# aras-p/UnityGaussianSplatting

Measured on AMD Instinct MI355X. Metric: Msplats/s rendered (sort+view+composite+resolve), bicycle-sized synthetic 6,131,954 splats, 1200x797, Medium; ms/frame in ms_per_step, higher is better.
Workload: dtype f32; 1 GPU; bicycle-sized synthetic 6,131,954 splats, 1200x797, Medium; sort_mode=visible_in_flight, frames_in_flight=2, frames_in_flight_impl=library, splats=6131954, views=1, views_per_rank=1, blend=exact, sort_nth_frame=1, tile_pairs_P=4376060, tile=32x16, visible_splats=1563698, parallelism=single GPU, rccl_ranks=0

## Files before the change

unitygaussiansplatting_amd/csrc/gs_common.h:

```cpp
#pragma once
#include <hip/hip_runtime.h>
#include <hip/hip_ext.h>
#include <stdint.h>
#include <stdio.h>
#include <string.h>
#include <utility>
#include <vector>

#include "../../include/gsplat_c.h"
#include "gs_device_math.h"
#include "gs_handles.h"
#include "gs_params.h"

#ifdef GS_CHAIN_PRIO
#define GS_CHAIN_PRIORITY() __builtin_amdgcn_s_setprio(GS_CHAIN_PRIO)
#else
#define GS_CHAIN_PRIORITY() do { } while (0)
#endif
#ifdef GS_VIEW_PRIO
#define GS_VIEW_PRIORITY() __builtin_amdgcn_s_setprio(GS_VIEW_PRIO)
#else
#define GS_VIEW_PRIORITY() do { } while (0)
#endif

namespace gs {

void set_error_detail(const char* fmt, ...);
int32_t fail(int32_t code, const char* what);
int32_t fail_hip(hipError_t e, const char* what, const char* file, int line);

#define GS_HIP(call)                                                        \
    do {                                                                    \
        hipError_t _e = (call);                                             \
        if (_e != hipSuccess) return gs::fail_hip(_e, #call, __FILE__, __LINE__); \
    } while (0)

#define GS_TRY(call)                    \
    do {                                \
        int32_t _r = (call);            \
        if (_r != GS_OK) return _r;     \
    } while (0)

constexpr int kBinThreads = 256;
constexpr int kBinItems = 8;
constexpr int kBinPart = kBinThreads * kBinItems;
constexpr uint32_t kBinTicketClasses = 16;
constexpr int kEvPerFrame = 28;

struct alignas(16) SplatRec {
    float cx, cy;
    float a1x, a1y;
    float a2x, a2y;
    uint32_t color0;
    uint32_t color1;
};
static_assert(sizeof(SplatRec) == 32, "SplatRec is 32 B");

struct ViewOutputs {
    gsm::ViewData* view;
    SplatRec* recs;
    uint2* rects;
    unsigned long long* visMask;
};
__host__ __device__ inline size_t vis_mask_words(uint32_t n) { return (((size_t)n + 63) / 64 + 7) & ~(size_t)7; }
__host__ __device__ inline uint8_t* wave_flags_of(unsigned long long* visMask, uint32_t n) { return (uint8_t*)(visMask + vis_mask_words(n)); }
__host__ __device__ inline size_t vis_alloc_bytes(uint32_t n) { return vis_mask_words(n) * 8 + ((size_t)n + 63) / 64 + 64; }

struct SortState {
    DevBuf<uint32_t> altKeys;
    DevBuf<uint32_t> altVals;
    DevBuf<uint32_t> status;
    DevBuf<unsigned long long> groupAgg;
    DevBuf<unsigned long long> groupIncl;
    uint32_t maxGroups = 0;
    uint32_t maxCount = 0;
    uint32_t maxParts = 0;
    uint32_t partMin = 8192;
    uint32_t histCopies = 1;
    uint32_t epoch = 0;
};

constexpr int kHistReplicas = 8;
constexpr int kHistStride = 4 * 256;
uint32_t hist_copies(int producerBlocks);
struct SortControl {
    uint32_t hist[kHistReplicas * kHistStride];
    uint32_t tickets[4][16 * 32];
    uint32_t error;
    uint32_t pad[3];
};

struct FrameReport {
    unsigned long long pairCount;
    uint32_t binError, pairSortError, visible, tileShape;
    uint32_t tieLongRuns, tieLongest;
};

constexpr int kVisHistory = 128;
constexpr uint32_t kVisMaxBlocks = 1024;
constexpr uint32_t kVisTieWaveMax = 64;
struct VisControl {
    uint32_t count;
    uint32_t tieLongRuns;
    uint32_t tieLongest;
    uint32_t error;
    uint32_t pad[28];
    uint32_t status[kVisMaxBlocks * 16];
};
constexpr uint32_t kVisStatusStride = 16;
struct TieHistory { float row[kVisHistory][4]; uint32_t depth; };
enum TieBase { TB_INDEX = 0,
               TB_RANK = 1,
               TB_POSITION = 2 };

struct alignas(16) PickRecord { float depth; uint32_t splat, tag, zero; };
static_assert(sizeof(PickRecord) == 16 && sizeof(PickRecord) == sizeof(gs_pick_record), "PickRecord is 16 B");
constexpr uint32_t kPickNoSplat = 0xFFFFFFFFu;
struct PickOut {
    PickRecord* rec;
    float tau;
    uint32_t tauHalfHi;
    uint32_t tag;
    uint32_t noDepth;
};

struct BinControl {
    unsigned long long pairCount;
    uint32_t pairCountClamped;
    uint32_t error;
    uint32_t tieLongRuns, tieLongest;
    uint32_t pad0[26];
    uint32_t visible;
    uint32_t pad1[31];
    uint32_t tickets[16 * 32];
};

}

struct gs_context {
    int device = 0;
    hipStream_t stream = nullptr;
    bool ownStream = false;
    hipStream_t aux = nullptr;
    bool overlap = false;
    gs::Event evOrder;
    bool viewGeneric = false;
    int sharedGpu = -1;
    bool counted = false;
    int cuCount = 0;
    hipDeviceProp_t props;
    std::vector<gs_context*> children;
    bool internalLane = false;
    bool sortBesideSiblings = false;
};
bool gs_shared_gpu(const gs_context* ctx);

struct gs_asset {
    gs_context* ctx = nullptr;
    gsm::AssetView view{};
    void* blobs[5] = {nullptr, nullptr, nullptr, nullptr, nullptr};
    gs::DevBuf<uint8_t> ownedBlobs[5];
    uint64_t sizes[5] = {0, 0, 0, 0, 0};
    bool owned = true;
};

struct gs_sorter {
    gs_context* ctx = nullptr;
    gs::SortState st;
    gs::DevBuf<gs::SortControl> control;
    gs::DevBuf<uint32_t> tmpKeys;
    gs::DevBuf<uint32_t> tmpVals;
};

struct gs_target {
    gs_context* ctx = nullptr;
    uint32_t width = 0, height = 0;
    gs::DevBuf<uint16_t> rgba16f;
    bool clearPending = false;
    const float* sceneDepth = nullptr;
    gs::DevBuf<float> sceneDepthOwned;
    gs::DevBuf<unsigned long long> zbuf;
    gs::DevBuf<float> resolved;
    gs::DevBuf<uint8_t> resolved8;
    static constexpr int kResolveRing = 64;
    std::vector<gs::Event> rev;
    bool profiling = false;
    int revCount = 0;
    gs::Event evLastUse;
    bool lastUseValid = false;
    gs::DevBuf<uint16_t> rgba16fAlt;
    gs::Event evLastUseAlt;
    bool lastUseValidAlt = false;
    bool exposed = false;
    gs::DevBuf<gs::PickRecord> pick;
    gs::DevBuf<gs::PickRecord> pickAlt;
    float pickTau = 0.5f;
};

struct gs_mask {
    gs_context* ctx = nullptr;
    uint32_t width = 0, height = 0, rowWords = 0;
    gs::DevBuf<uint32_t> words;
    gs::DevBuf<float> xy;
    gs::PinnedBuf<float> xyHost;
    gs::Event xyCopied;
    bool xyCopyPending = false;
    uint32_t xyCap = 0;
    gs::PinnedBuf<uint32_t> wordsHost;
    gs::Event wordsCopied;
    bool wordsCopyPending = false;
};

namespace gs {
struct RendererSettings {
    int blendMode = 0;
    int renderMode = 0;
    float pointDisplaySize = 3.0f;
    bool alwaysWriteView = false;
    bool kernelTiming = false;
// ... 243 lines not shown
```

unitygaussiansplatting_amd/csrc/gs_device_math.h:

```cpp
#pragma once
#include <stdint.h>

#if defined(__HIPCC__)
#include <hip/hip_runtime.h>
#include <hip/hip_fp16.h>
#define GS_HD __host__ __device__ __forceinline__
#else
#include <cmath>
#include <cstring>
#define GS_HD inline
#endif

#ifndef GS_CULL_EXTENT
#define GS_CULL_EXTENT 2.8285f
#endif

namespace gsm {

struct AssetView {
    const uint8_t* pos;
    const uint8_t* other;
    const uint8_t* color;
    const uint8_t* sh;
    const uint8_t* chunk;
// ... 874 lines not shown
            return s;
        };
        auto MUL = [](float w, const RGB& s) -> RGB { return { F2{ w, w } * s.rg, w * s.b }; };
        auto FMA = [](float w, const RGB& s, const RGB& acc) -> RGB { return { fma2(F2{ w, w }, s.rg, acc.rg), fmaf(w, s.b, acc.b) }; };
        {
            const RGB s1v = SHK(1), s2v = SHK(2), s3v = SHK(3);
            RGB t = MUL(dy, RGB{ -s1v.rg, -s1v.b });
            t = FMA(dz, s2v, t);
            t = FMA(dx, RGB{ -s3v.rg, -s3v.b }, t);
            rg = fma2(F2{ GS_SH_C1, GS_SH_C1 }, t.rg, rg); b = fmaf(GS_SH_C1, t.b, b);
        }
        if (P.shOrder >= 2) {
            const float xx = dx * dx, yy = dy * dy, zz = dz * dz;
            const float xy = dx * dy, yz = dy * dz, xz = dx * dz;
            {
                const float b4 = 1.0925484f * xy, b5 = -1.0925484f * yz, b6 = 0.3153916f * (fmaf(2.0f, zz, -xx) - yy),
                            b7 = -1.0925484f * xz, b8 = 0.5462742f * (xx - yy);
                RGB acc = MUL(b4, SHK(4));
                acc = FMA(b5, SHK(5), acc);
                acc = FMA(b6, SHK(6), acc);
                acc = FMA(b7, SHK(7), acc);
                acc = FMA(b8, SHK(8), acc);
                rg += acc.rg; b += acc.b;
            }
            if (P.shOrder >= 3) {
                const float b9 = (-0.5900436f * dy) * fmaf(3.0f, xx, -yy);
                const float b10 = (2.8906114f * xy) * dz;
                const float b11 = (-0.4570458f * dy) * (fmaf(4.0f, zz, -xx) - yy);
                const float b12 = (0.3731763f * dz) * (fmaf(2.0f, zz, -3.0f * xx) - 3.0f * yy);
                const float b13 = (-0.4570458f * dx) * (fmaf(4.0f, zz, -xx) - yy);
                const float b14 = (1.4453057f * dz) * (xx - yy);
                const float b15 = (-0.5900436f * dx) * fmaf(-3.0f, yy, xx);
                RGB acc = MUL(b9, SHK(9));
                acc = FMA(b10, SHK(10), acc);
                acc = FMA(b11, SHK(11), acc);
                acc = FMA(b12, SHK(12), acc);
                acc = FMA(b13, SHK(13), acc);
                acc = FMA(b14, SHK(14), acc);
                acc = FMA(b15, SHK(15), acc);
                rg += acc.rg; b += acc.b;
            }
        }
    }
    float r = rg.x, g = rg.y;
    r = fmaxf(r, 0.0f); g = fmaxf(g, 0.0f); b = fmaxf(b, 0.0f);
    view.color[0] = (f32tof16(r) << 16) | f32tof16(g);
    view.color[1] = (f32tof16(b) << 16) | (view.color[1] & 0xffffu);
}

template <class SHSource>
GS_HD ViewData CalcViewDataT(const AssetView& a, const FrameConsts& P, const EditView& E, uint32_t idx, SHSource& shsrc) {
    ViewPartial vp;
    CalcViewGeom(a, P, E, idx, vp);
    if (vp.front) CalcViewColor(a, P, idx, vp, shsrc);
    return vp.view;
}

GS_HD ViewData CalcViewData(const AssetView& a, const FrameConsts& P, const EditView& E, uint32_t idx) {
    SHFromBlob src;
    return CalcViewDataT(a, P, E, idx, src);
}

GS_HD void PixRange(float c, float e, float size, int& lo, int& hi) {
    float flo = ceilf((c - e) - 0.5f), fhi = floorf((c + e) - 0.5f);
    flo = fmaxf(flo, 0.0f); fhi = fminf(fhi, size - 1.0f);
    if (!(flo <= fhi)) { lo = 1; hi = 0; return; }
    lo = (int)flo; hi = (int)fhi;
}

constexpr uint32_t kAlphaThresholdBits = 0x3B808081u;
constexpr uint32_t kAlphaWindow = 16u;
constexpr uint32_t kAlphaWindowLo = kAlphaThresholdBits - kAlphaWindow / 2u;
GS_HD float Exp2Det(float y) {
    const float n = rintf(y);
    const float f = y - n;
    float p = 1.525273380405984e-05f;
    p = fmaf(p, f, 1.5403530393381608e-04f);
    p = fmaf(p, f, 1.3333558146428443e-03f);
    p = fmaf(p, f, 9.618129107628477e-03f);
    p = fmaf(p, f, 5.550410866482158e-02f);
    p = fmaf(p, f, 2.402265069591007e-01f);
    p = fmaf(p, f, 6.931471805599453e-01f);
    p = fmaf(p, f, 1.0f);
    return ldexpf(p, (int)n);
}
GS_HD float DecideAlpha(float alphaNative, float y, float a, bool& live) {
    const uint32_t u = f2u(alphaNative) - kAlphaWindowLo;
    if (u < kAlphaWindow) {
        const float ad = fminf(fmaxf(Exp2Det(y) * a, 0.0f), 1.0f);
        live = ad >= u2f(kAlphaThresholdBits);
        return ad;
    }
    live = (int32_t)u >= (int32_t)kAlphaWindow;
    return alphaNative;
}

constexpr uint32_t kSelRingLoBits = 0x3CE0E0E1u;
constexpr uint32_t kSelRingHiBits = 0x3D20A0A1u;
GS_HD bool SplatSelected(const EditView& E, uint32_t idx) { return E.selectedBits && ((E.selectedBits[idx >> 5] >> (idx & 31u)) & 1u); }
constexpr uint32_t kSelectedAlphaHalf = 0xBC00u;
GS_HD bool SelectedNearThreshold(float eNative) {
    const uint32_t b = f2u(eNative), h = kAlphaWindow / 2u;
    return (b - (kAlphaThresholdBits - h) < kAlphaWindow) | (b - (kSelRingLoBits - h) < kAlphaWindow) | (b - (kSelRingHiBits - h) < kAlphaWindow);
}
GS_HD float DecideSelected(float eNative, float y, bool& ring, bool& live, bool windowed = true) {
    float e = eNative;
    if (windowed && SelectedNearThreshold(eNative)) e = Exp2Det(y);
    float alpha = e;
    ring = false;
    if (e > u2f(kSelRingLoBits)) {
        if (e < u2f(kSelRingHiBits)) { alpha = 1.0f; ring = true; }
        alpha = fminf(fmaxf(alpha + 0.3f, 0.0f), 1.0f);
    }
    live = alpha >= u2f(kAlphaThresholdBits);
    return alpha;
}
GS_HD bool SelectedFragment(float eNative, float y, float r, float g, float b, float* out4, bool windowed = true) {
    bool ring, live;
    const float alpha = DecideSelected(eNative, y, ring, live, windowed);
    if (ring) { r = 1.0f; g = 0.0f; b = 1.0f; }
    r = fmaf(0.5f, 1.0f - r, r); g = fmaf(0.5f, 0.0f - g, g); b = fmaf(0.5f, 1.0f - b, b);
    out4[0] = r * alpha; out4[1] = g * alpha; out4[2] = b * alpha; out4[3] = alpha;
    return live;
}

GS_HD float LogDetCore(uint32_t u, int ebias) {
    float e = (float)((int)(u >> 23) + ebias);
    float m = u2f((u & 0x7fffffu) | 0x3f800000u);
    if (m > 1.41421356f) { m *= 0.5f; e += 1.0f; }
    const float t = (m - 1.0f) / (m + 1.0f);
    const float t2 = t * t;
    const float p = fmaf(t2, fmaf(t2, fmaf(t2, 1.0f / 7.0f, 0.2f), 1.0f / 3.0f), 1.0f);
    return fmaf(e, 0.69314718f, (2.0f * t) * p);
}
GS_HD float LogDet(float x) { return LogDetCore(f2u(x), -127); }

GS_HD bool BlockMayTouch(float bcx, float bcy, float half, float cx, float cy, float u1x, float u1y, float u2x, float u2y, float r2) {
    const float dx = bcx - cx, dy = bcy - cy;
    const float d1 = fabsf(fmaf(dy, u1y, dx * u1x)) - half * (fabsf(u1x) + fabsf(u1y));
    const float d2 = fabsf(fmaf(dy, u2y, dx * u2x)) - half * (fabsf(u2x) + fabsf(u2y));
    const float m1 = fmaxf(d1, 0.0f), m2 = fmaxf(d2, 0.0f);
    return (m1 <= 2.001f) && (m2 <= 2.001f) && (fmaf(m2, m2, m1 * m1) <= r2);
}

struct SplatFootprint {
    float cx, cy;
    int x0, x1, y0, y1;
};
GS_HD void PackPixelRect(const SplatFootprint& fp, uint32_t& rx, uint32_t& ry) {
    rx = (uint32_t)fp.x0 | ((uint32_t)fp.y0 << 16);
    ry = (uint32_t)(fp.x1 + 1) | ((uint32_t)(fp.y1 + 1) << 16);
}

GS_HD bool PrepareSplat(const ViewData& v, float W, float H, float nearClip, float farClip, SplatFootprint& fp) {
    fp.x0 = 1; fp.x1 = 0; fp.y0 = 1; fp.y1 = 0; fp.cx = 0.0f; fp.cy = 0.0f;
    const float w = v.pos[3];
    const float a = f16tof32(v.color[1]);
    const int drawable = (int)(w > 0.0f) & (int)(w >= nearClip) & (int)(w <= farClip) & (int)finite32(v.axis1[0]) & (int)finite32(v.axis1[1]) &
                         (int)finite32(v.axis2[0]) & (int)finite32(v.axis2[1]) & (int)(a >= 1.0f / 255.0f);
    if (!drawable) return false;
    const float invw = 1.0f / w;
    const float cx = fmaf(0.5f * (v.pos[0] * invw), W, 0.5f * W);
    const float cy = fmaf(-0.5f * (v.pos[1] * invw), H, 0.5f * H);
    const float a1x = v.axis1[0], a1y = v.axis1[1], a2x = v.axis2[0], a2y = v.axis2[1];
    const float d1 = dot2f(a1x, a1y, a1x, a1y), d2 = dot2f(a2x, a2y, a2x, a2y);
    const int inv1ok = (int)((f2u(d1) - 0x00200001u) <= (0x7f800000u - 0x00200001u)), inv2ok = (int)((f2u(d2) - 0x00200001u) <= (0x7f800000u - 0x00200001u));
    fp.cx = cx; fp.cy = cy;
    if (!((int)finite32(cx) & (int)finite32(cy) & inv1ok & inv2ok)) return false;
    const float exr = 2.0f * (fabsf(a1x) + fabsf(a2x)), eyr = 2.0f * (fabsf(a1y) + fabsf(a2y));
    const float slack = 0.01f;
    int x0, x1, y0, y1;
    PixRange(fp.cx, exr + slack, W, x0, x1);
    PixRange(fp.cy, eyr + slack, H, y0, y1);
    if (x0 > x1 || y0 > y1) return false;
    const float r2 = fmaf(LogDet(255.0f * a), 1.0001f, 1.0e-3f);
    const float rr = sqrtf(fmaxf(r2, 0.0f));
    const float exe = rr * sqrtf(dot2f(a1x, a2x, a1x, a2x)), eye = rr * sqrtf(dot2f(a1y, a2y, a1y, a2y));
    PixRange(fp.cx, fminf(exr, exe) + slack, W, x0, x1);
    PixRange(fp.cy, fminf(eyr, eye) + slack, H, y0, y1);
    if (x0 > x1 || y0 > y1) return true;
    fp.x0 = x0; fp.x1 = x1; fp.y0 = y0; fp.y1 = y1;
    return true;
}

GS_HD bool PrepareSplatHighlight(const ViewData& v, bool selected, float W, float H, float nearClip, float farClip, SplatFootprint& fp) {
    ViewData o = v;
    if (selected) o.color[1] = (v.color[1] & 0xffff0000u) | 0x3C00u;
    return PrepareSplat(o, W, H, nearClip, farClip, fp);
}
GS_HD uint32_t RecordColor1(uint32_t color1, bool selected) { return selected ? ((color1 & 0xffff0000u) | kSelectedAlphaHalf) : color1; }

GS_HD float LogDetFull(float x) {
    const uint32_t u = f2u(x);
    if (u >= 0x7f800000u) {
        if ((u << 1) == 0u) return u2f(0xff800000u);
        if (u == 0x7f800000u) return x;
        return u2f(0x7fc00000u);
    }
    if (u == 0u) return u2f(0xff800000u);
    if (u < 0x00800000u) return LogDetCore(f2u(x * 8388608.0f), -150);
    return LogDetCore(u, -127);
}

struct SplatFull { V3 pos; V4 rot; V3 scale; float opacity; V3 col; V3 sh[15]; };
GS_HD void LoadSplatDataFull(const AssetView& a, uint32_t idx, uint32_t ci, const V3& pos, SplatFull& s) {
    s.pos = pos;
    uint32_t otherStride = 4 + vecStride(a.scaleFmt);
    if (a.shFmt > 3) otherStride += 2;
    const uint64_t otherAddr = (uint64_t)idx * otherStride;
    s.rot = DecodeRotation(LoadUInt(a.other, otherAddr));
    s.scale = LoadVec(a.other, otherAddr + 4, a.scaleFmt);
    V4 col = LoadColorTexel(a, idx);
    uint32_t shIndex = idx;
    if (a.shFmt > 3) shIndex = LoadUShort(a.other, otherAddr + otherStride - 2);
    const uint8_t* sp = a.sh + (uint64_t)shIndex * shStrideOf(a.shFmt);
#pragma unroll
    for (int k = 0; k < 15; ++k) s.sh[k] = LoadSH(sp, a.shFmt, k + 1);
    if (ci < a.chunkCount) {
        const ChunkRaw ck = LoadChunk(a.chunk, ci);
        s.scale.x = lerpf(f16tof32(ck.w[10]), f16tof32(ck.w[10] >> 16), s.scale.x);
        s.scale.y = lerpf(f16tof32(ck.w[11]), f16tof32(ck.w[11] >> 16), s.scale.y);
        s.scale.z = lerpf(f16tof32(ck.w[12]), f16tof32(ck.w[12] >> 16), s.scale.z);
        s.scale.x *= s.scale.x; s.scale.y *= s.scale.y; s.scale.z *= s.scale.z;
        s.scale.x *= s.scale.x; s.scale.y *= s.scale.y; s.scale.z *= s.scale.z;
        s.scale.x *= s.scale.x; s.scale.y *= s.scale.y; s.scale.z *= s.scale.z;
        col.x = lerpf(f16tof32(ck.w[0]), f16tof32(ck.w[0] >> 16), col.x);
        col.y = lerpf(f16tof32(ck.w[1]), f16tof32(ck.w[1] >> 16), col.y);
        col.z = lerpf(f16tof32(ck.w[2]), f16tof32(ck.w[2] >> 16), col.z);
        col.w = lerpf(f16tof32(ck.w[3]), f16tof32(ck.w[3] >> 16), col.w);
        col.w = InvSquareCentered01(col.w);
        if (a.shFmt > 0 && a.shFmt <= 3) {
            const V3 lo = { f16tof32(ck.w[13]), f16tof32(ck.w[14]), f16tof32(ck.w[15]) };
            const V3 hi = { f16tof32(ck.w[13] >> 16), f16tof32(ck.w[14] >> 16), f16tof32(ck.w[15] >> 16) };
#pragma unroll
            for (int k = 0; k < 15; ++k) s.sh[k] = { lerpf(lo.x, hi.x, s.sh[k].x), lerpf(lo.y, hi.y, s.sh[k].y), lerpf(lo.z, hi.z, s.sh[k].z) };
        }
    }
    s.opacity = col.w;
    s.col = { col.x, col.y, col.z };
}

struct SHRot { float sh1[3][3]; float sh2[5][5]; float sh3[7][7]; };
GS_HD float SHRotP(const float (*r1)[3], const float* prev, int l, int i, int a, int n) {
    const int w = 2 * l - 1, c = l - 1;
    const float* row = prev + (a + c) * w;
    if (n == l) return r1[i + 1][2] * row[2 * c] - r1[i + 1][0] * row[0];
    if (n == -l) return r1[i + 1][2] * row[0] + r1[i + 1][0] * row[2 * c];
    return r1[i + 1][1] * row[n + c];
}
struct SHRotSum {
    const float (*r1)[3]; const float* prev; int l, n; float acc; bool any;
    GS_HD void add(double c64, int i, int a) {
        const float c = (float)c64;
        if (c == 0.0f) return;
        const float t = c * SHRotP(r1, prev, l, i, a, n);
        acc = any ? acc + t : t;
        any = true;
    }
};
GS_HD void SHRotBand(const float (*r1)[3], const float* prev, int l, float* out) {
    const double sqrt2 = sqrt(2.0);
    for (int m = -l; m <= l; ++m)
        for (int n = -l; n <= l; ++n) {
            const int am = m < 0 ? -m : m, an = n < 0 ? -n : n;
            const double d = an < l ? (double)((l + n) * (l - n)) : (double)(2 * l * (2 * l - 1));
            const double u = sqrt((double)((l + m) * (l - m)) / d);
            const double v = sqrt((double)((l + am - 1) * (l + am)) / d) * 0.5;
            const double w = -(sqrt((double)((l - am - 1) * (l - am)) / d) * 0.5);
            SHRotSum s = { r1, prev, l, n, 0.0f, false };
            s.add(u, 0, m);
            if (m == 0) { s.add(-(v * sqrt2), 1, 1); s.add(-(v * sqrt2), -1, -1); }
            else if (m > 0) { s.add(m == 1 ? v * sqrt2 : v, 1, m - 1); if (m != 1) s.add(-v, -1, -m + 1); s.add(w, 1, m + 1); s.add(w, -1, -m - 1); }
            else { if (m != -1) s.add(v, 1, m + 1); s.add(m == -1 ? v * sqrt2 : v, -1, -m - 1); s.add(w, 1, m - 1); s.add(-w, -1, -m + 1); }
            out[(m + l) * (2 * l + 1) + (n + l)] = s.any ? s.acc : 0.0f;
        }
}
GS_HD void SHRotMatrix(const float* o2w, float (*m)[3]) {
    for (int r = 0; r < 3; ++r) {
        const float x = o2w[r * 4], y = o2w[r * 4 + 1], z = o2w[r * 4 + 2];
        const float inv = 1.0f / sqrtf((x * x + y * y) + z * z);
        m[r][0] = x * inv; m[r][1] = y * inv; m[r][2] = z * inv;
    }
}
GS_HD void CalcSHRot(const float* o2w, SHRot& R) {
    float m[3][3];
    SHRotMatrix(o2w, m);
    R.sh1[0][0] = m[1][1]; R.sh1[0][1] = -m[1][2]; R.sh1[0][2] = m[1][0];
    R.sh1[1][0] = -m[2][1]; R.sh1[1][1] = m[2][2]; R.sh1[1][2] = -m[2][0];
    R.sh1[2][0] = m[0][1]; R.sh1[2][1] = -m[0][2]; R.sh1[2][2] = m[0][0];
    SHRotBand(R.sh1, &R.sh1[0][0], 2, &R.sh2[0][0]);
    SHRotBand(R.sh1, &R.sh2[0][0], 3, &R.sh3[0][0]);
}

struct ExportXform { uint32_t bake; float o2w[12]; float rot[4]; float scale[3]; SHRot sh; };

GS_HD V3 SHDotRow(const V3* v, const float* f, int n) {
    V3 r = { v[0].x * f[0], v[0].y * f[0], v[0].z * f[0] };
    for (int k = 1; k < n; ++k) { r.x = r.x + v[k].x * f[k]; r.y = r.y + v[k].y * f[k]; r.z = r.z + v[k].z * f[k]; }
    return r;
}

GS_HD V4 BakeQuat(const float* rot, const V4& q) { return QuatMul({ rot[0], rot[1], rot[2], rot[3] }, q); }
GS_HD V3 BakeScale(const V3& s, const float* scale) { return { s.x * fabsf(scale[0]), s.y * fabsf(scale[1]), s.z * fabsf(scale[2]) }; }
template <int N> GS_HD void RotateSHBand(const V3* in, const float (*f)[N], V3* out) {
#pragma unroll
    for (int k = 0; k < N; ++k) out[k] = SHDotRow(in, f[k], N);
}
GS_HD void BakeSplatTransform(SplatFull& s, const float* m, const float* rot, const float* scale, const SHRot& sh) {
    const V3 pos = s.pos;
    s.pos = { mrow(m, 0, pos.x, pos.y, pos.z), mrow(m, 1, pos.x, pos.y, pos.z), mrow(m, 2, pos.x, pos.y, pos.z) };
    if (scale[0] < 0.0f) { s.rot.y = -s.rot.y; s.rot.z = -s.rot.z; }
    if (scale[1] < 0.0f) { s.rot.x = -s.rot.x; s.rot.z = -s.rot.z; }
    if (scale[2] < 0.0f) { s.rot.x = -s.rot.x; s.rot.y = -s.rot.y; }
    s.rot = BakeQuat(rot, s.rot);
    s.scale = BakeScale(s.scale, scale);
    V3 out[15];
    RotateSHBand<3>(s.sh, sh.sh1, out);
    RotateSHBand<5>(s.sh + 3, sh.sh2, out + 3);
    RotateSHBand<7>(s.sh + 8, sh.sh3, out + 8);
#pragma unroll
    for (int k = 0; k < 15; ++k) s.sh[k] = out[k];
}

struct EditRigid { float q[4]; float s; SHRot sh; };
GS_HD uint32_t EditRigidRotateWord(const EditRigid& G, uint32_t mouseDown) {
    return EncodeQuatToNorm10(PackSmallest3Rotation(BakeQuat(G.q, DecodeRotation(mouseDown))));
}
GS_HD V3 EditRigidScale(const EditRigid& G, const V3& mouseDown) {
    const float s3[3] = { G.s, G.s, G.s };
    return BakeScale(mouseDown, s3);
}
template <int N> GS_HD void EditRigidSHBand(const float* src, float* dst, const float (*f)[N], int first) {
    V3 in[N], out[N];
#pragma unroll
    for (int k = 0; k < N; ++k) in[k] = { src[3 * (first + k)], src[3 * (first + k) + 1], src[3 * (first + k) + 2] };
    RotateSHBand<N>(in, f, out);
#pragma unroll
    for (int k = 0; k < N; ++k) { dst[3 * (first + k)] = out[k].x; dst[3 * (first + k) + 1] = out[k].y; dst[3 * (first + k) + 2] = out[k].z; }
}
GS_HD void EditRigidRotateSH(const EditRigid& G, const float* src, float* dst) {
    EditRigidSHBand<3>(src, dst, G.sh.sh1, 0);
// ... 671 lines not shown
```

unitygaussiansplatting_amd/csrc/gs_view.hip:

```cpp
#include "gs_common.h"

namespace gs {

namespace {

template <int FMT> struct SHFromLds {
    const uint32_t* rec;
    __device__ __forceinline__ void begin(const uint8_t*, uint32_t) {}
    __device__ __forceinline__ uint32_t half_at(int h) const { return (rec[h >> 1] >> ((h & 1) * 16)) & 0xffffu; }
    __device__ __forceinline__ gsm::V3 load(int k) const {
        if (FMT == 0) return { gsm::u2f(rec[(k - 1) * 3]), gsm::u2f(rec[(k - 1) * 3 + 1]), gsm::u2f(rec[(k - 1) * 3 + 2]) };
        if (FMT == 2) return gsm::Dec_11_10_11(rec[k - 1]);
        if (FMT == 3) return gsm::Dec_5_6_5(half_at(k - 1));
        return { gsm::f16tof32(half_at((k - 1) * 3)), gsm::f16tof32(half_at((k - 1) * 3 + 1)), gsm::f16tof32(half_at((k - 1) * 3 + 2)) };
    }
    __device__ __forceinline__ gsm::RGB load_rgb(int k) const {
        if (FMT == 3) {
            const uint32_t e = half_at(k - 1);
            return { gsm::F2{ (float)(e & 31), (float)((e >> 5) & 63) } * gsm::F2{ GS_R31, GS_R63 }, (float)((e >> 11) & 31) * GS_R31 };
        }
        const gsm::V3 v = load(k);
        return { gsm::F2{ v.x, v.y }, v.z };
    }
};

constexpr int sh_rec_dwords(int fmt) { return fmt == 0 ? 48 : (fmt == 1 ? 24 : (fmt == 2 ? 15 : 8)); }
constexpr int cmax(int a, int b) { return a > b ? a : b; }

struct EditViewPlain { const uint32_t* deletedBits; const uint32_t* cutouts; uint32_t cutoutCount; };
template <bool HL> struct EditArg { typedef EditViewPlain type; };
template <> struct EditArg<true> { typedef gsm::EditView type; };
__device__ __forceinline__ gsm::EditView edit_view_of(const EditViewPlain& p) { gsm::EditView e; e.deletedBits = p.deletedBits; e.cutouts = p.cutouts; e.cutoutCount = p.cutoutCount; return e; }
__device__ __forceinline__ gsm::EditView edit_view_of(const gsm::EditView& e) { return e; }

template <int SHMODE, bool FULL, bool HL, class F = gsm::RuntimeFormats>
__global__ __launch_bounds__(256) void calc_view_kernel(gsm::AssetView a, gsm::FrameConsts P, typename EditArg<HL>::type Earg, ViewOutputs O) {
    const gsm::EditView E = edit_view_of(Earg);
    GS_VIEW_PRIORITY();
    gsm::ViewData* __restrict__ out = O.view;
    SplatRec* __restrict__ recs = O.recs;
    uint2* __restrict__ rects = O.rects;
    unsigned long long* __restrict__ visMask = O.visMask;
    constexpr int REC = sh_rec_dwords(SHMODE < 4 ? SHMODE : 3);
    constexpr int STRIDE = REC | 1;
    constexpr int SH_DW = SHMODE < 4 ? 256 * STRIDE : 0;
    constexpr int NVEC = (REC * 256 / 4 + 255) / 256;
    __shared__ uint4 s_stage[cmax(SH_DW, FULL ? 256 * 10 : 4) / 4 + 1];
    __shared__ int s_any;
    uint32_t* s_dw = (uint32_t*)s_stage;
    const uint32_t base = blockIdx.x * 256u;
    const uint32_t idx = base + threadIdx.x;
    const uint32_t cnt = min(256u, a.n - base);
    const uint32_t totalDw = cnt * (uint32_t)REC, totalVec = totalDw >> 2;
    const uint32_t* shSrc = (const uint32_t*)(a.sh + (size_t)base * (REC * 4));

    uint4 shv[SHMODE < 4 ? NVEC : 1];
    uint32_t shTail = 0;
    auto sh_issue = [&]() {
#pragma unroll
        for (int it = 0; it < NVEC; ++it) {
            const uint32_t j = (uint32_t)it * 256u + threadIdx.x;
            shv[it] = make_uint4(0u, 0u, 0u, 0u);
            if (j < totalVec) shv[it] = ((const uint4*)shSrc)[j];
        }
        if ((totalDw & 3u) && threadIdx.x < (totalDw & 3u)) shTail = shSrc[(totalVec << 2) + threadIdx.x];
    };
    auto sh_park = [&]() {
#pragma unroll
        for (int it = 0; it < NVEC; ++it) {
            const uint32_t j = (uint32_t)it * 256u + threadIdx.x;
            if (j < totalVec) {
                const uint32_t d = j << 2;
                const uint32_t v[4] = { shv[it].x, shv[it].y, shv[it].z, shv[it].w };
                if (REC % 4 == 0) {
                    const uint32_t r = d / (uint32_t)REC, o = d - r * (uint32_t)REC;
#pragma unroll
                    for (int c = 0; c < 4; ++c) s_dw[r * STRIDE + o + c] = v[c];
                } else {
#pragma unroll
                    for (int c = 0; c < 4; ++c) { const uint32_t dd = d + c, r = dd / (uint32_t)REC; s_dw[r * STRIDE + (dd - r * (uint32_t)REC)] = v[c]; }
                }
            }
        }
        if ((totalDw & 3u) && threadIdx.x < (totalDw & 3u)) { const uint32_t dd = (totalVec << 2) + threadIdx.x, r = dd / (uint32_t)REC; s_dw[r * STRIDE + (dd - r * (uint32_t)REC)] = shTail; }
    };
    auto shade = [&](gsm::ViewPartial& vp) {
        if (SHMODE < 4) {
            SHFromLds<SHMODE < 4 ? SHMODE : 3> src;
            src.rec = s_dw + threadIdx.x * STRIDE;
            gsm::CalcViewColor<F>(a, P, idx, vp, src);
        } else {
            gsm::SHFromBlob src;
            gsm::CalcViewColor<F>(a, P, idx, vp, src);
        }
    };

    gsm::ViewPartial vp;
    gsm::SplatFootprint fp;
    uint2 rect = make_uint2(0u, 0u);
    bool visible = false;
    bool selected = false;
    const bool shStaged = SHMODE < 4;

    if (FULL) {
        if (shStaged) { sh_issue(); sh_park(); __syncthreads(); }
        if (idx < a.n) {
            gsm::CalcViewGeom<F>(a, P, E, idx, vp);
            if (vp.front) shade(vp);
            bool ok;
            if (HL) {
                selected = vp.front && gsm::SplatSelected(E, idx);
                ok = gsm::PrepareSplatHighlight(vp.view, selected, P.screenW, P.screenH, P.nearClip, P.farClip, fp);
            } else {
                ok = gsm::PrepareSplat(vp.view, P.screenW, P.screenH, P.nearClip, P.farClip, fp);
            }
            visible = ok && fp.x0 <= fp.x1;
        }
    } else {
        if (P.cullOn && F::chunked(a, blockIdx.x)) {
            const uint32_t m = gsm::ChunkCornerOutside(a, P, blockIdx.x, threadIdx.x & 7u);
            bool outside = false;
#pragma unroll
            for (int pl = 0; pl < 6; ++pl) outside = outside || __all((m >> pl) & 1u);
            if (outside) {
                if (idx < a.n) rects[idx] = make_uint2(0u, 0u);
                if ((threadIdx.x & 63u) == 0u && idx < a.n) visMask[idx >> 6] = 0ull;
                if ((threadIdx.x & 63u) == 0u && idx < a.n) wave_flags_of(visMask, a.n)[idx >> 6] = 0u;
                return;
            }
        }
        if (threadIdx.x == 0) s_any = 0;
        if (idx < a.n) {
            gsm::CalcViewGeom<F>(a, P, E, idx, vp, true, true);
            bool ok;
            if (HL) {
                selected = vp.front && !vp.culled && gsm::SplatSelected(E, idx);
                ok = vp.front && !vp.culled && gsm::PrepareSplatHighlight(vp.view, selected, P.screenW, P.screenH, P.nearClip, P.farClip, fp);
            } else {
                ok = vp.front && !vp.culled && gsm::PrepareSplat(vp.view, P.screenW, P.screenH, P.nearClip, P.farClip, fp);
            }
            visible = ok && fp.x0 <= fp.x1;
        }
        __syncthreads();
        if (__any(visible) && (threadIdx.x & 63u) == 0u) s_any = 1;
        __syncthreads();
        if (s_any) {
            if (shStaged) { sh_issue(); sh_park(); __syncthreads(); }
            if (visible) shade(vp);
        }
    }

    if (idx < a.n) {
        if (visible) {
            gsm::PackPixelRect(fp, rect.x, rect.y);
            uint4* rp = (uint4*)(recs + idx);
            rp[0] = make_uint4(gsm::f2u(fp.cx), gsm::f2u(fp.cy), gsm::f2u(vp.view.axis1[0]), gsm::f2u(vp.view.axis1[1]));
            rp[1] = make_uint4(gsm::f2u(vp.view.axis2[0]), gsm::f2u(vp.view.axis2[1]), vp.view.color[0], HL ? gsm::RecordColor1(vp.view.color[1], selected) : vp.view.color[1]);
        }
        rects[idx] = rect;
    }
    const unsigned long long vb = __ballot(visible);
    if ((threadIdx.x & 63u) == 0u && (idx < a.n)) visMask[idx >> 6] = vb;
    if ((threadIdx.x & 63u) == 0u && (idx < a.n)) wave_flags_of(visMask, a.n)[idx >> 6] = vb != 0ull ? 1u : 0u;
    if (!FULL) return;

    if (shStaged) __syncthreads();
    if (idx < a.n) {
        const gsm::ViewData& v = vp.view;
        uint32_t* o = s_dw + threadIdx.x * 10;
        o[0] = gsm::f2u(v.pos[0]); o[1] = gsm::f2u(v.pos[1]); o[2] = gsm::f2u(v.pos[2]); o[3] = gsm::f2u(v.pos[3]);
        o[4] = gsm::f2u(v.axis1[0]); o[5] = gsm::f2u(v.axis1[1]); o[6] = gsm::f2u(v.axis2[0]); o[7] = gsm::f2u(v.axis2[1]);
        o[8] = v.color[0]; o[9] = v.color[1];
    }
    __syncthreads();
    {
        const uint32_t dwords = cnt * 10u;
        uint32_t* g = (uint32_t*)(out + base);
        const uint32_t vec = dwords / 4u;
        for (uint32_t j = threadIdx.x; j < vec; j += 256u) ((uint4*)g)[j] = s_stage[j];
        for (uint32_t j = vec * 4u + threadIdx.x; j < dwords; j += 256u) g[j] = s_dw[j];
    }
}

typedef gsm::AssetFormats<0, 0, 0, 0, 0> FormatsVeryHigh;
typedef gsm::AssetFormats<1, 1, 1, 2, 1> FormatsHigh;
typedef gsm::AssetFormats<2, 2, 2, 3, 1> FormatsMedium;
typedef gsm::AssetFormats<2, 3, 2, 6, 1> FormatsLow;
typedef gsm::AssetFormats<2, 3, 3, 8, 1> FormatsVeryLow;

}

template <bool FULL>
static void launch_calc_view(int mode, uint32_t grid, hipStream_t st, const gsm::AssetView& a, const gsm::FrameConsts& c, const gsm::EditView& e,
                             const ViewOutputs& o) {
    const EditViewPlain ep = { e.deletedBits, e.cutouts, e.cutoutCount };
#define GS_LAUNCH_VIEW(M) do { if (e.selectedBits) hipLaunchKernelGGL((calc_view_kernel<M, FULL, true>), dim3(grid), dim3(256), 0, st, a, c, e, o); \
                               else hipLaunchKernelGGL((calc_view_kernel<M, FULL, false>), dim3(grid), dim3(256), 0, st, a, c, ep, o); } while (0)
    switch (mode) {
        case 0: GS_LAUNCH_VIEW(0); break;
        case 1: GS_LAUNCH_VIEW(1); break;
        case 2: GS_LAUNCH_VIEW(2); break;
        case 3: GS_LAUNCH_VIEW(3); break;
        default: GS_LAUNCH_VIEW(4); break;
    }
#undef GS_LAUNCH_VIEW
}

template <int SHMODE, class F>
static bool try_calc_view_preset(int mode, uint32_t grid, hipStream_t st, const gsm::AssetView& a, const gsm::FrameConsts& c, const EditViewPlain& ep, const ViewOutputs& o) {
    if (mode != SHMODE || a.posFmt != (uint32_t)F::kPos || a.scaleFmt != (uint32_t)F::kScale || a.colorFmt != (uint32_t)F::kColor || a.shFmt != (uint32_t)F::kSH) return false;
    if (F::kChunked ? a.chunkCount < grid : a.chunkCount != 0u) return false;
    hipLaunchKernelGGL((calc_view_kernel<SHMODE, false, false, F>), dim3(grid), dim3(256), 0, st, a, c, ep, o);
    return true;
}
static bool launch_calc_view_preset(int mode, uint32_t grid, hipStream_t st, const gsm::AssetView& a, const gsm::FrameConsts& c, const gsm::EditView& e, const ViewOutputs& o) {
    const EditViewPlain ep = { e.deletedBits, e.cutouts, e.cutoutCount };
    return try_calc_view_preset<0, FormatsVeryHigh>(mode, grid, st, a, c, ep, o) || try_calc_view_preset<2, FormatsHigh>(mode, grid, st, a, c, ep, o) ||
           try_calc_view_preset<3, FormatsMedium>(mode, grid, st, a, c, ep, o) || try_calc_view_preset<4, FormatsLow>(mode, grid, st, a, c, ep, o) ||
           try_calc_view_preset<4, FormatsVeryLow>(mode, grid, st, a, c, ep, o);
}

int32_t enqueue_calc_view(gs_context* ctx, const gsm::AssetView& a, const gs_frame_params* p, const gsm::EditView& e, const ViewOutputs& out, bool full) {
    gsm::FrameConsts c;
    flatten_params(p, c);
    const uint32_t grid = (a.n + 255u) / 256u;
    const int mode = (a.shFmt <= 3 && (((uintptr_t)a.sh) & 15u) == 0 && p->sh_order >= 1) ? (int)a.shFmt : 4;
    const bool presetAllowed = !full && !e.selectedBits && !ctx->viewGeneric;
    if (presetAllowed && launch_calc_view_preset(mode, grid, ctx->stream, a, c, e, out)) {}
    else if (full) launch_calc_view<true>(mode, grid, ctx->stream, a, c, e, out);
    else launch_calc_view<false>(mode, grid, ctx->stream, a, c, e, out);
    GS_HIP(hipGetLastError());
    return GS_OK;
}

}
```

Baseline: 16250 Msplats/s.

## Precompute chunk frustum culling in a separate kernel and drop coarse pixel-range test

```diff
diff --git a/unitygaussiansplatting_amd/csrc/gs_common.h b/unitygaussiansplatting_amd/csrc/gs_common.h
--- a/unitygaussiansplatting_amd/csrc/gs_common.h
+++ b/unitygaussiansplatting_amd/csrc/gs_common.h
@@ -64,7 +64,10 @@
 };
 __host__ __device__ inline size_t vis_mask_words(uint32_t n) { return (((size_t)n + 63) / 64 + 7) & ~(size_t)7; }
 __host__ __device__ inline uint8_t* wave_flags_of(unsigned long long* visMask, uint32_t n) { return (uint8_t*)(visMask + vis_mask_words(n)); }
-__host__ __device__ inline size_t vis_alloc_bytes(uint32_t n) { return vis_mask_words(n) * 8 + ((size_t)n + 63) / 64 + 64; }
+__host__ __device__ inline size_t wave_flag_bytes(uint32_t n) { return (((size_t)n + 63) / 64 + 15) & ~(size_t)15; }
+__host__ __device__ inline size_t chunk_dead_bytes(uint32_t n) { return (((size_t)n + 255) / 256 + 15) & ~(size_t)15; }
+__host__ __device__ inline uint8_t* chunk_dead_of(unsigned long long* visMask, uint32_t n) { return wave_flags_of(visMask, n) + wave_flag_bytes(n); }
+__host__ __device__ inline size_t vis_alloc_bytes(uint32_t n) { return vis_mask_words(n) * 8 + wave_flag_bytes(n) + chunk_dead_bytes(n) + 64; }
 
 struct SortState {
     DevBuf<uint32_t> altKeys;
diff --git a/unitygaussiansplatting_amd/csrc/gs_device_math.h b/unitygaussiansplatting_amd/csrc/gs_device_math.h
--- a/unitygaussiansplatting_amd/csrc/gs_device_math.h
+++ b/unitygaussiansplatting_amd/csrc/gs_device_math.h
@@ -1050,6 +1050,7 @@
     ry = (uint32_t)(fp.x1 + 1) | ((uint32_t)(fp.y1 + 1) << 16);
 }
 
+template <bool LEAN = false>
 GS_HD bool PrepareSplat(const ViewData& v, float W, float H, float nearClip, float farClip, SplatFootprint& fp) {
     fp.x0 = 1; fp.x1 = 0; fp.y0 = 1; fp.y1 = 0; fp.cx = 0.0f; fp.cy = 0.0f;
     const float w = v.pos[3];
@@ -1068,9 +1069,11 @@
     const float exr = 2.0f * (fabsf(a1x) + fabsf(a2x)), eyr = 2.0f * (fabsf(a1y) + fabsf(a2y));
     const float slack = 0.01f;
     int x0, x1, y0, y1;
-    PixRange(fp.cx, exr + slack, W, x0, x1);
-    PixRange(fp.cy, eyr + slack, H, y0, y1);
-    if (x0 > x1 || y0 > y1) return false;
+    if (!LEAN) {
+        PixRange(fp.cx, exr + slack, W, x0, x1);
+        PixRange(fp.cy, eyr + slack, H, y0, y1);
+        if (x0 > x1 || y0 > y1) return false;
+    }
     const float r2 = fmaf(LogDet(255.0f * a), 1.0001f, 1.0e-3f);
     const float rr = sqrtf(fmaxf(r2, 0.0f));
     const float exe = rr * sqrtf(dot2f(a1x, a2x, a1x, a2x)), eye = rr * sqrtf(dot2f(a1y, a2y, a1y, a2y));
@@ -1081,10 +1084,11 @@
     return true;
 }
 
+template <bool LEAN = false>
 GS_HD bool PrepareSplatHighlight(const ViewData& v, bool selected, float W, float H, float nearClip, float farClip, SplatFootprint& fp) {
     ViewData o = v;
     if (selected) o.color[1] = (v.color[1] & 0xffff0000u) | 0x3C00u;
-    return PrepareSplat(o, W, H, nearClip, farClip, fp);
+    return PrepareSplat<LEAN>(o, W, H, nearClip, farClip, fp);
 }
 GS_HD uint32_t RecordColor1(uint32_t color1, bool selected) { return selected ? ((color1 & 0xffff0000u) | kSelectedAlphaHalf) : color1; }
 
diff --git a/unitygaussiansplatting_amd/csrc/gs_view.hip b/unitygaussiansplatting_amd/csrc/gs_view.hip
--- a/unitygaussiansplatting_amd/csrc/gs_view.hip
+++ b/unitygaussiansplatting_amd/csrc/gs_view.hip
@@ -117,12 +117,9 @@
             visible = ok && fp.x0 <= fp.x1;
         }
     } else {
-        if (P.cullOn && F::chunked(a, blockIdx.x)) {
-            const uint32_t m = gsm::ChunkCornerOutside(a, P, blockIdx.x, threadIdx.x & 7u);
-            bool outside = false;
-#pragma unroll
-            for (int pl = 0; pl < 6; ++pl) outside = outside || __all((m >> pl) & 1u);
-            if (outside) {
+        if (F::kChunked != 0 && P.cullOn) {
+            const bool dead = ((((const uint32_t*)chunk_dead_of(visMask, a.n))[blockIdx.x >> 2] >> ((blockIdx.x & 3u) * 8u)) & 0xffu) != 0u;
+            if (dead) {
                 if (idx < a.n) rects[idx] = make_uint2(0u, 0u);
                 if ((threadIdx.x & 63u) == 0u && idx < a.n) visMask[idx >> 6] = 0ull;
                 if ((threadIdx.x & 63u) == 0u && idx < a.n) wave_flags_of(visMask, a.n)[idx >> 6] = 0u;
@@ -135,9 +132,9 @@
             bool ok;
             if (HL) {
                 selected = vp.front && !vp.culled && gsm::SplatSelected(E, idx);
-                ok = vp.front && !vp.culled && gsm::PrepareSplatHighlight(vp.view, selected, P.screenW, P.screenH, P.nearClip, P.farClip, fp);
+                ok = vp.front && !vp.culled && gsm::PrepareSplatHighlight<true>(vp.view, selected, P.screenW, P.screenH, P.nearClip, P.farClip, fp);
             } else {
-                ok = vp.front && !vp.culled && gsm::PrepareSplat(vp.view, P.screenW, P.screenH, P.nearClip, P.farClip, fp);
+                ok = vp.front && !vp.culled && gsm::PrepareSplat<true>(vp.view, P.screenW, P.screenH, P.nearClip, P.farClip, fp);
             }
             visible = ok && fp.x0 <= fp.x1;
         }
@@ -187,6 +184,15 @@
 typedef gsm::AssetFormats<2, 2, 2, 3, 1> FormatsMedium;
 typedef gsm::AssetFormats<2, 3, 2, 6, 1> FormatsLow;
 typedef gsm::AssetFormats<2, 3, 3, 8, 1> FormatsVeryLow;
+
+__global__ __launch_bounds__(256) void chunk_cull_kernel(gsm::AssetView a, gsm::FrameConsts P, uint8_t* __restrict__ chunkDead, uint32_t grid) {
+    const uint32_t t = blockIdx.x * 256u + threadIdx.x;
+    const uint32_t ci = t >> 3, corner = t & 7u;
+    uint32_t m = 0u;
+    if (ci < grid && ci < a.chunkCount) m = gsm::ChunkCornerOutside(a, P, ci, corner);
+    m &= __shfl_xor(m, 1); m &= __shfl_xor(m, 2); m &= __shfl_xor(m, 4);
+    if (corner == 0u && ci < grid) chunkDead[ci] = m != 0u ? 1u : 0u;
+}
 
 }
 
@@ -225,6 +231,8 @@
     flatten_params(p, c);
     const uint32_t grid = (a.n + 255u) / 256u;
     const int mode = (a.shFmt <= 3 && (((uintptr_t)a.sh) & 15u) == 0 && p->sh_order >= 1) ? (int)a.shFmt : 4;
+    if (a.chunkCount == 0u) c.cullOn = 0u;
+    if (!full && c.cullOn) hipLaunchKernelGGL(chunk_cull_kernel, dim3((grid * 8u + 255u) / 256u), dim3(256), 0, ctx->stream, a, c, chunk_dead_of(out.visMask, a.n), grid);
     const bool presetAllowed = !full && !e.selectedBits && !ctx->viewGeneric;
     if (presetAllowed && launch_calc_view_preset(mode, grid, ctx->stream, a, c, e, out)) {}
     else if (full) launch_calc_view<true>(mode, grid, ctx->stream, a, c, e, out);
```

New measurement: 16140 Msplats/s. Within noise of the previous version (-0.7%).
